# ZooMEISTER/vickers-hardness-Unet

Hardware: AMD Instinct MI355X
Metric: 512x512 images/sec (train fwd+bwd) (higher is better)
Workload: dtype bf16

## Files before the change

include/vk_unet.h:

```cpp
#ifndef VK_UNET_H
#define VK_UNET_H

#include <stddef.h>
#include <stdint.h>

#ifdef __cplusplus
extern "C" {
#endif

#define VK_ABI_VERSION 1
#define VK_STATS_REPLICAS 32

typedef enum { VK_F32 = 0, VK_BF16 = 1, VK_F16 = 2 } vk_dtype;

enum { VK_OK = 0, VK_ERR_ARG = -1, VK_ERR_STATE = -2, VK_ERR_UNSUPPORTED = -3 };

int vk_version(void);
const char* vk_last_error_string(void);
int vk_has_gfx950_code(void);
int vk_probe_mfma_rate(int iters, int waves_per_simd, float* sink, double* flops_out, void* stream);
int vk_set_reserved_cus(int n);
int vk_debug_hold_cus(int workgroups, int threads, int lds_bytes, int microseconds, const void* traffic, size_t traffic_bytes,
                      float* sink, void* stream);

// ... 331 lines not shown
int vk_unet_encoder(const vk_unet* h);
void vk_unet_destroy(vk_unet* h);
int vk_unet_set_side_stream(vk_unet* h, int enable);
int vk_unet_num_tensors(const vk_unet* h);
int vk_unet_tensor_info(const vk_unet* h, int index, vk_tensor_info* out);
int64_t vk_unet_param_numel(const vk_unet* h);
int64_t vk_unet_buffer_numel(const vk_unet* h);
int64_t vk_unet_workspace_bytes(const vk_unet* h);
int vk_unet_num_buckets(const vk_unet* h);
int vk_unet_bucket_range(const vk_unet* h, int bucket, int64_t* elem_begin, int64_t* elem_end);

int vk_unet_bind(vk_unet* h, float* params, float* grads, float* bn_buffers, int64_t* nbt, void* workspace,
                 size_t workspace_bytes);
int vk_unet_refresh_weights(vk_unet* h, void* stream);

int vk_unet_forward(vk_unet* h, const float* x, float* logits, int training, void* stream);
int vk_unet_loss(vk_unet* h, const float* logits, const float* target, float* loss_out, float grad_scale,
                 float w_bce, float w_dice, void* stream);
#define VK_LOSS_BINARY 0
#define VK_LOSS_MULTILABEL 1
#define VK_LOSS_MULTICLASS 2
int vk_unet_loss_ex(vk_unet* h, int mode, const void* logits, const void* target, float* loss_out, float grad_scale, float w_ce,
                    float w_dice, void* stream);
int vk_unet_loss_cfg(vk_unet* h, const vk_seg_loss_cfg* cfg, const void* logits, const void* target, float* loss_out,
                     float grad_scale, void* stream);
int vk_unet_loss_lovasz(vk_unet* h, const vk_seg_loss_cfg* seg_cfg, const vk_lovasz_cfg* lovasz_cfg, float w_lovasz, const void* logits,
                        const void* target, void* workspace, size_t workspace_bytes, float* loss_out, float grad_scale, void* stream);
int vk_unet_backward(vk_unet* h, const float* dlogits, int stage_begin, int stage_end, void* stream);
int vk_unet_set_trainable(vk_unet* h, const uint8_t* flags, int n);
int vk_unet_set_bn_frozen(vk_unet* h, const uint8_t* flags, int n);
// ... 19 lines not shown
```

vickers-hardness-unet_amd/_lib.py:

```python
from __future__ import annotations

import ctypes as C
import os
import subprocess
from pathlib import Path

PKG_DIR = Path(__file__).resolve().parent
LIB_PATH = Path(os.environ["VK_LIB"]) if os.environ.get("VK_LIB") else PKG_DIR / "libvkunet.so"
CSRC = PKG_DIR / "csrc"

VK_F32, VK_BF16, VK_F16 = 0, 1, 2
VK_LOSS_BINARY, VK_LOSS_MULTILABEL, VK_LOSS_MULTICLASS = 0, 1, 2
VK_ENC_RESNET18, VK_ENC_RESNET34, VK_ENC_RESNET50 = 18, 34, 50
VK_ADAMW_MAX_GROUPS = 8
VK_NORM_L2, VK_NORM_INF = 0, 1
VK_TILE_MAX_ORIGINS, VK_TILE_MAX_SIDE = 64, 4096
VK_BLEND_PROB, VK_BLEND_LOGIT = 0, 1


class VkError(RuntimeError):
    pass


class vk_src(C.Structure):
    _fields_ = [("ptr", C.c_void_p), ("C", C.c_int), ("up", C.c_int), ("scale", C.c_void_p),
                ("shift", C.c_void_p), ("relu", C.c_int)]


class vk_conv_desc(C.Structure):
    _fields_ = [("dtype", C.c_int), ("N", C.c_int), ("H", C.c_int), ("W", C.c_int), ("Ho", C.c_int),
# ... 44 lines not shown
    _fields_ = [("struct_size", C.c_uint32), ("mode", C.c_int32), ("terms", C.c_uint32), ("has_ignore", C.c_int32),
                ("ignore_index", C.c_int32), ("w_pix", C.c_float), ("w_focal", C.c_float), ("w_dice", C.c_float),
                ("w_jaccard", C.c_float), ("w_tversky", C.c_float), ("pix_smooth", C.c_float), ("pix_denom_valid", C.c_int32),
                ("has_pos_weight", C.c_int32), ("pos_weight", C.c_float * 16), ("focal_has_alpha", C.c_int32),
                ("focal_alpha", C.c_float), ("focal_gamma", C.c_float),
                ("dice_smooth", C.c_float), ("dice_eps", C.c_float), ("dice_log", C.c_int32), ("dice_classes", C.c_uint32),
                ("jaccard_smooth", C.c_float), ("jaccard_eps", C.c_float), ("jaccard_log", C.c_int32), ("jaccard_classes", C.c_uint32),
                ("tversky_smooth", C.c_float), ("tversky_eps", C.c_float), ("tversky_log", C.c_int32), ("tversky_classes", C.c_uint32),
                ("tversky_alpha", C.c_float), ("tversky_beta", C.c_float), ("tversky_gamma", C.c_float),
                ("w_mcc", C.c_float), ("mcc_eps", C.c_float)]


class vk_lovasz_cfg(C.Structure):
    _fields_ = [("struct_size", C.c_uint32), ("mode", C.c_int32), ("per_image", C.c_int32), ("has_ignore", C.c_int32),
                ("ignore_index", C.c_int32)]


class vk_adamw_group(C.Structure):
    _fields_ = [("lr", C.c_float), ("beta1", C.c_float), ("beta2", C.c_float), ("eps", C.c_float), ("weight_decay", C.c_float)]


class vk_unet_config(C.Structure):
    _fields_ = [("N", C.c_int), ("size", C.c_int), ("dtype", C.c_int), ("training", C.c_int), ("width", C.c_int)]


class vk_tensor_info(C.Structure):
    _fields_ = [("name", C.c_char * 96), ("kind", C.c_int), ("dims", C.c_int * 4), ("ndim", C.c_int),
                ("offset", C.c_int64), ("numel", C.c_int64)]


# ... 89 lines not shown
    "vk_unet_create_ex": (ci, [P(vk_unet_config), ci, P(vp)]),
    "vk_unet_num_classes": (ci, [vp]),
    "vk_unet_create_enc": (ci, [P(vk_unet_config), ci, ci, P(vp)]),
    "vk_unet_encoder": (ci, [vp]),
    "vk_unet_destroy": (None, [vp]),
    "vk_unet_set_side_stream": (ci, [vp, ci]),
    "vk_unet_num_tensors": (ci, [vp]),
    "vk_unet_tensor_info": (ci, [vp, ci, P(vk_tensor_info)]),
    "vk_unet_param_numel": (i64, [vp]),
    "vk_unet_buffer_numel": (i64, [vp]),
    "vk_unet_workspace_bytes": (i64, [vp]),
    "vk_unet_num_buckets": (ci, [vp]),
    "vk_unet_bucket_range": (ci, [vp, ci, P(i64), P(i64)]),
    "vk_unet_bind": (ci, [vp, vp, vp, vp, vp, vp, sz]),
    "vk_unet_refresh_weights": (ci, [vp, vp]),
    "vk_unet_forward": (ci, [vp, vp, vp, ci, vp]),
    "vk_unet_loss": (ci, [vp, vp, vp, vp, cf, cf, cf, vp]),
    "vk_unet_loss_ex": (ci, [vp, ci, vp, vp, vp, cf, cf, cf, vp]),
    "vk_unet_loss_cfg": (ci, [vp, P(vk_seg_loss_cfg), vp, vp, vp, cf, vp]),
    "vk_unet_loss_lovasz": (ci, [vp, P(vk_seg_loss_cfg), P(vk_lovasz_cfg), cf, vp, vp, vp, sz, vp, cf, vp]),
    "vk_unet_backward": (ci, [vp, vp, ci, ci, vp]),
    "vk_unet_set_trainable": (ci, [vp, P(C.c_uint8), ci]),
    "vk_unet_set_bn_frozen": (ci, [vp, P(C.c_uint8), ci]),
    "vk_unet_set_input_grad": (ci, [vp, vp]),
    "vk_unet_zero_grad": (ci, [vp, vp]),
    "vk_unet_debug_tensor": (ci, [vp, C.c_char_p, P(vp), P(ci * 4)]),
    "vk_comm_unique_id": (ci, [vp]),
    "vk_comm_init": (ci, [ci, ci, vp, P(vp)]),
    "vk_comm_world": (ci, [vp]),
    "vk_allreduce_bucket": (ci, [vp, vp, sz, vp]),
# ... 76 lines not shown
```

vickers-hardness-unet_amd/csrc/elementwise.hip:

```cpp
#include <math.h>

#include "vk_common.h"

namespace vk {

static inline int grid_for(size_t work_items, int block = 256, int max_blocks = 256 * 16) {
  size_t b = (work_items + block - 1) / block;
  if (b > (size_t)max_blocks) b = max_blocks;
  if (b < 1) b = 1;
  return (int)b;
}

constexpr int kWideC = 2048;
static inline int channel_grid(int blocks, int cv) {
  int g = cv, r = 256;
  while (r) { const int t = g % r; g = r; r = t; }
  const int m = cv / g;
  return (blocks + m - 1) / m * m;
}

template <typename T>
__global__ void k_input_transform(int N, int H, int W, const float* __restrict__ x, T* __restrict__ x4) {
  const size_t HW = (size_t)H * W;
  const float* xn = x + (size_t)blockIdx.y * 3 * HW;
// ... 1584 lines not shown
  dim3 grid(grid_for(n)), block(256);
  if (!lowp_copy || lowp_dtype == VK_F32) {
    hipLaunchKernelGGL(k_adamw_dev<float>, grid, block, 0, st, n, param, grad, exp_avg, exp_avg_sq, lr, beta1, beta2, eps, weight_decay,
                       (const float*)scratch4, (float*)nullptr);
  } else if (lowp_dtype == VK_BF16) {
    hipLaunchKernelGGL(k_adamw_dev<bf16_t>, grid, block, 0, st, n, param, grad, exp_avg, exp_avg_sq, lr, beta1, beta2, eps, weight_decay,
                       (const float*)scratch4, (bf16_t*)lowp_copy);
  } else {
    hipLaunchKernelGGL(k_adamw_dev<f16_t>, grid, block, 0, st, n, param, grad, exp_avg, exp_avg_sq, lr, beta1, beta2, eps, weight_decay,
                       (const float*)scratch4, (f16_t*)lowp_copy);
  }
  VK_CHECK_HIP(hipGetLastError());
  return VK_OK;
}

extern "C" int vk_adamw_segment_blocks(int n_segments, const int64_t* seg, int32_t* blocks, int capacity) {
  VK_CHECK_ARG(n_segments >= 1 && seg && (capacity >= 0), "vk_adamw_segment_blocks: bad argument");
  int64_t rows = 0;
  for (int s = 0; s < n_segments; ++s) {
    const int64_t b = seg[3 * s], e = seg[3 * s + 1];
    VK_CHECK_ARG(0 <= b && b < e && seg[3 * s + 2] >= 0, "vk_adamw_segment_blocks: bad segment %d [%lld, %lld)", s, (long long)b, (long long)e);
    const int64_t chunks = (e - b + VK_ADAMW_SEGMENT_CHUNK - 1) / VK_ADAMW_SEGMENT_CHUNK;
    for (int64_t c = 0; c < chunks; ++c, ++rows) {
      VK_CHECK_ARG(rows < (1 << 30), "vk_adamw_segment_blocks: too many blocks");
      if (blocks && rows < capacity) {
        blocks[2 * rows] = s;
        blocks[2 * rows + 1] = (int32_t)c;
      }
    }
  }
// ... 36 lines not shown
```

vickers-hardness-unet_amd/csrc/engine.hip:

```cpp
#include <stdarg.h>
#include <stdio.h>
#include <stdlib.h>
#include <string.h>

#include <algorithm>
#include <atomic>
#include <map>
#include <mutex>
#include <string>
#include <vector>

#include "vk_common.h"

namespace vkh {
static thread_local char g_err[512] = "";
void set_error(const char* fmt, ...) {
  va_list ap;
  va_start(ap, fmt);
  vsnprintf(g_err, sizeof(g_err), fmt, ap);
  va_end(ap);
}

struct ProfRec {
  std::string tag;
// ... 221 lines not shown
template <typename T>
__global__ void k_cast_ranges(const CastRange* __restrict__ tab, const float* __restrict__ src, T* __restrict__ dst) {
  const CastRange r = tab[blockIdx.y];
  for (int64_t i = blockIdx.x * (int64_t)blockDim.x + threadIdx.x; i < r.count; i += (int64_t)gridDim.x * blockDim.x)
    st1(dst + r.begin + i, src[r.begin + i]);
}

template <typename T>
__global__ void k_pack_stem(const float* __restrict__ w, T* __restrict__ wp) {
  const int i = blockIdx.x * blockDim.x + threadIdx.x;
  if (i >= 64 * 7 * 32) return;
  const int j = i % 32, r = (i / 32) % 7, k = i / (32 * 7);
  const int s = j >> 2, c = j & 3;
  const float v = (s < 7 && c < 3) ? w[((k * 7 + r) * 7 + s) * 3 + c] : 0.f;
  st1(wp + i, v);
}

struct BnEvalEntry {
  int64_t g_off, b_off, rm_off, rv_off, out_off;
  int C, pad_;
};
__global__ void k_bn_eval_all(const BnEvalEntry* __restrict__ tab, const float* __restrict__ params, const float* __restrict__ bufs,
                              float* __restrict__ arena, float eps) {
  const BnEvalEntry e = tab[blockIdx.x];
  for (int c = threadIdx.x; c < e.C; c += blockDim.x) {
    const float invstd = (float)(1.0 / sqrt((double)bufs[e.rv_off + c] + (double)eps));
    const float sc = params[e.g_off + c] * invstd;
    arena[e.out_off + c] = sc;
    arena[e.out_off + e.C + c] = params[e.b_off + c] - bufs[e.rm_off + c] * sc;
  }
// ... 160 lines not shown
  struct WPlan {
    bool built = false;
    int target = 0, n = 0;
    unsigned version = 0;
    vk::WgradBatchPlan plan;
  };
  std::vector<WItem> pending;
  WPlan wplans[kMaxStages][2];
  size_t off_tab_wbatch = 0;
  std::vector<PackEntry> pack_tab;
  std::vector<CastRange> cast_tab;
  size_t off_tab_cast = 0;
  size_t off_gscratch = 0;
  size_t off_sloss = 0, sloss_bytes = 0;
  size_t off_mloss = 0, mloss_bytes = 0;
  std::vector<BnEvalEntry> bn_tab;
  std::map<std::string, std::pair<void*, std::vector<int>>> debug;

  int N() const { return cfg.N; }
};

namespace {

size_t align_up(size_t v, size_t a) { return (v + a - 1) / a * a; }

bool need_from(const vk_unet* h, int rank) { return h->last_rank >= rank; }
bool trains(const vk_unet* h, int t) { return h->trainable[(size_t)t] != 0; }
bool frozen(const vk_unet* h, const BnL& b) { return (h->bn_frozen_fwd >> b.idx) & 1ull; }
bool bn_sums_needed(const vk_unet* h, const BnL& b) { return !frozen(h, b) || trains(h, b.g_t) || trains(h, b.b_t); }
float* grad_or_sink(vk_unet* h, int t, int64_t off, int sink_off) {
  return trains(h, t) ? h->grads + off : (float*)(h->ws + h->off_gscratch) + sink_off;
}
float* dgamma_of(vk_unet* h, const BnL& b) { return grad_or_sink(h, b.g_t, b.g_off, 0); }
float* dbeta_of(vk_unet* h, const BnL& b) { return grad_or_sink(h, b.b_t, b.b_off, h->sink_c); }

// ... 250 lines not shown
  h->off_wstem = take(64 * 7 * 32 * eb);
  h->off_wslab = tr ? take(kEngineSlabBytes) : 0;
  h->off_tab_wbatch = tr ? take((size_t)kMaxStages * 2 * VK_WGRAD_BATCH_TABLE_BYTES) : 0;
  h->splitk_bytes = (!tr && (size_t)N * S * SW <= 4u * 512 * 512) ? VK_SPLITK_WORKSPACE_BYTES : 0;
  h->off_splitk = h->splitk_bytes ? take(h->splitk_bytes) : 0;
  h->off_tab_pack = take(h->convs.size() * sizeof(PackEntry));
  h->off_tab_cast = take(h->convs.size() * sizeof(CastRange));
  h->off_tab_bn = take(h->bns.size() * sizeof(BnEvalEntry));
  h->off_gscratch = tr ? take(grad_scratch_floats(h) * sizeof(float)) : 0;
  if (h->classes > 1) {
    h->mloss_bytes = vk_multi_loss_workspace_bytes(N, h->classes, S * SW);
    h->off_mloss = take(h->mloss_bytes);
  }
  h->sloss_bytes = vk_seg_loss_workspace_bytes(N, h->classes, S * SW);
  h->off_sloss = take(h->sloss_bytes);
  h->ws_bytes = off;
}

void assign_pointers(vk_unet* h) {
  char* ws = h->ws;
  h->debug.clear();
  const int N = h->cfg.N;
  for (size_t i = 0; i < h->convs.size(); ++i) {
    ConvL& c = h->convs[i];
    if ((int)i == h->head_conv) continue;
    c.z = ws + h->off_z[i];
    c.g = h->cfg.training ? ws + h->off_g[i] : nullptr;
    h->debug["z:" + c.name] = {c.z, {N, c.Hout, c.Wout, c.K}};
    if (c.g) h->debug["g:" + c.name] = {c.g, {N, c.Hout, c.Wout, c.K}};
  }
// ... 174 lines not shown
  VK_CHECK_ARG(h && out && index >= 0 && index < (int)h->infos.size(), "vk_unet_tensor_info: bad index %d", index);
  *out = h->infos[index];
  return VK_OK;
}
extern "C" int64_t vk_unet_param_numel(const vk_unet* h) { return h ? h->n_params : 0; }
extern "C" int64_t vk_unet_buffer_numel(const vk_unet* h) { return h ? h->n_bufs : 0; }
extern "C" int64_t vk_unet_workspace_bytes(const vk_unet* h) { return h ? (int64_t)h->ws_bytes : 0; }
extern "C" int vk_unet_num_buckets(const vk_unet* h) { return h ? (int)h->buckets.size() : 0; }
extern "C" int vk_unet_bucket_range(const vk_unet* h, int bucket, int64_t* b, int64_t* e) {
  VK_CHECK_ARG(h && b && e && bucket >= 0 && bucket < (int)h->buckets.size(), "vk_unet_bucket_range: bad bucket %d", bucket);
  *b = h->buckets[bucket].first;
  *e = h->buckets[bucket].second;
  return VK_OK;
}

extern "C" int vk_unet_bind(vk_unet* h, float* params, float* grads, float* bn_buffers, int64_t* nbt, void* workspace,
                            size_t workspace_bytes) {
  VK_CHECK_ARG(h && params && bn_buffers && nbt && workspace, "vk_unet_bind: null argument");
  VK_CHECK_ARG(!h->cfg.training || grads, "vk_unet_bind: a training plan needs a gradient buffer");
  VK_CHECK_ARG(workspace_bytes >= h->ws_bytes, "vk_unet_bind: workspace too small (%zu < %zu)", workspace_bytes, h->ws_bytes);
  VK_CHECK_ARG(((uintptr_t)workspace & 255) == 0 && ((uintptr_t)params & 15) == 0, "vk_unet_bind: buffers must be 256-byte (workspace) / 16-byte (params) aligned");
  h->params = params; h->grads = grads; h->bufs = bn_buffers; h->nbt = nbt; h->ws = (char*)workspace;
  for (auto& st_ : h->wplans) { st_[0].built = false; st_[1].built = false; }
  h->pending.clear();
  assign_pointers(h);
  h->halo_tab.clear();
  {
    auto plain = [&](int C) { vk_src s = null_src(); s.ptr = h->ws; s.C = C; return s; };
    auto fwd_uses = [&](ConvL& c, int C0, int C1, int up) {
      vk_src s0 = plain(C0), s1 = C1 ? plain(C1) : null_src();
      s0.up = up;
      vk_conv_desc d = conv_desc(h, c, s0, s1);
      return vk_conv_uses_halo_pack(&d) != 0;
    };
    for (size_t i = 0; i < h->convs.size(); ++i) {
      ConvL& c = h->convs[i];
      c.halo_fwd = c.halo_dg = false;
      if ((int)i == h->stem_conv || (int)i == h->head_conv) continue;
      c.halo_fwd = fwd_uses(c, c.Cin, 0, 0);
    }
    for (DecL& d : h->decs) {
      ConvL& c = h->convs[d.conv1];
      c.halo_fwd = fwd_uses(c, d.Cup, d.Cskip, 1);
    }
    for (size_t i = 0; i < h->convs.size(); ++i) {
      ConvL& c = h->convs[i];
      if (c.wd_off >= 0 && h->cfg.training) {
        vk_conv_desc d;
        d.dtype = h->cfg.dtype;
        d.N = h->cfg.N; d.H = c.Hout; d.W = c.Wout; d.Ho = c.Hin; d.Wo = c.Win;
        d.K = c.Cin; d.R = c.R; d.S = c.R; d.stride = c.stride; d.pad = c.pad; d.transposed = 1;
        d.src0 = plain(c.K);
        d.src1 = null_src();
        c.halo_dg = vk_conv_uses_halo_pack(&d) != 0;
      }
      HaloPackEntry e;
      e.src = c.w_off; e.pad_ = 0;
      if (c.halo_fwd) {
        e.dst = (int64_t)(h->off_wh + (size_t)c.w_off * h->eb); e.rows = c.K; e.red = c.Cin; e.transposed = 0;
        h->halo_tab.push_back(e);
      }
      if (c.halo_dg) {
        e.dst = (int64_t)(h->off_wd + (size_t)c.wd_off * h->eb); e.rows = c.Cin; e.red = c.K; e.transposed = 1;
        h->halo_tab.push_back(e);
      }
    }
  }
  h->pack_tab.clear();
  for (size_t i = 0; i < h->convs.size(); ++i) {
    const ConvL& c = h->convs[i];
    if (c.wd_off < 0 || c.halo_dg) continue;
    PackEntry e;
    e.src = c.w_off; e.dst = c.wd_off; e.K = c.K; e.RS = c.R * c.R; e.C = c.Cin; e.pad_ = 0;
    h->pack_tab.push_back(e);
  }
  h->cast_tab.clear();
  for (size_t i = 0; i < h->convs.size(); ++i) {
    const ConvL& c = h->convs[i];
    if ((int)i == h->stem_conv || (int)i == h->head_conv || c.halo_fwd) continue;
    h->cast_tab.push_back(CastRange{c.w_off, (int64_t)c.K * c.Cin * c.R * c.R});
  }
  h->bn_tab.clear();
  for (const BnL& b : h->bns) {
    BnEvalEntry e;
    e.g_off = b.g_off; e.b_off = b.b_off; e.rm_off = b.rm_off; e.rv_off = b.rv_off; e.out_off = b.arena_off; e.C = b.C; e.pad_ = 0;
    h->bn_tab.push_back(e);
  }
  if (!h->pack_tab.empty())
    VK_CHECK_HIP(hipMemcpy(h->ws + h->off_tab_pack, h->pack_tab.data(), h->pack_tab.size() * sizeof(PackEntry), hipMemcpyHostToDevice));
  if (!h->halo_tab.empty())
    VK_CHECK_HIP(hipMemcpy(h->ws + h->off_tab_halo, h->halo_tab.data(), h->halo_tab.size() * sizeof(HaloPackEntry), hipMemcpyHostToDevice));
  if (!h->cast_tab.empty())
    VK_CHECK_HIP(hipMemcpy(h->ws + h->off_tab_cast, h->cast_tab.data(), h->cast_tab.size() * sizeof(CastRange), hipMemcpyHostToDevice));
  VK_CHECK_HIP(hipMemcpy(h->ws + h->off_tab_bn, h->bn_tab.data(), h->bn_tab.size() * sizeof(BnEvalEntry), hipMemcpyHostToDevice));
  if (h->cfg.training && !h->side && getenv("VK_SIDE_STREAM")) RET_IF(vk_unet_set_side_stream(h, 1));
  h->bound = true;
  return VK_OK;
}

template <typename T>
static int refresh_t(vk_unet* h, hipStream_t st) {
  vkh::ProfScope ps_("weights_repack", st, 0.0, (double)h->n_params * (4.0 + 2.0 * sizeof(T)));
  if (sizeof(T) != 4 && !h->cast_tab.empty())
    hipLaunchKernelGGL(k_cast_ranges<T>, dim3(16, (unsigned)h->cast_tab.size()), dim3(256), 0, st, (const CastRange*)(h->ws + h->off_tab_cast),
                       h->params, (T*)(h->ws + h->off_wf));
  if (h->cfg.training && !h->pack_tab.empty())
    hipLaunchKernelGGL(k_pack_dgrad<T>, dim3(64, (unsigned)h->pack_tab.size()), dim3(256), 0, st,
                       (const PackEntry*)(h->ws + h->off_tab_pack), h->params, (T*)(h->ws + h->off_wd));
  if (!h->halo_tab.empty())
// ... 2 lines not shown
  hipLaunchKernelGGL(k_pack_stem<T>, dim3((64 * 7 * 32 + 255) / 256), dim3(256), 0, st,
                     h->params + h->convs[h->stem_conv].w_off, (T*)(h->ws + h->off_wstem));
  VK_CHECK_HIP(hipGetLastError());
  return VK_OK;
}

extern "C" int vk_unet_refresh_weights(vk_unet* h, void* stream) {
  VK_CHECK_ARG(h && h->bound, "vk_unet_refresh_weights: plan not bound");
  hipStream_t st = (hipStream_t)stream;
  switch (h->cfg.dtype) {
    case VK_F32: return refresh_t<float>(h, st);
    case VK_BF16: return refresh_t<bf16_t>(h, st);
    case VK_F16: return refresh_t<f16_t>(h, st);
  }
  return VK_ERR_ARG;
}

extern "C" int vk_unet_set_side_stream(vk_unet* h, int enable) {
  VK_CHECK_ARG(h, "vk_unet_set_side_stream: null plan");
  if (enable && !h->side && h->cfg.training) {
    VK_CHECK_HIP(hipStreamCreateWithFlags(&h->side, hipStreamNonBlocking));
    VK_CHECK_HIP(hipEventCreateWithFlags(&h->ev_fork, hipEventDisableTiming));
    VK_CHECK_HIP(hipEventCreateWithFlags(&h->ev_join, hipEventDisableTiming));
  } else if (!enable && h->side) {
    VK_CHECK_HIP(hipStreamSynchronize(h->side));
    (void)hipEventDestroy(h->ev_fork);
    (void)hipEventDestroy(h->ev_join);
    (void)hipStreamDestroy(h->side);
    h->side = nullptr;
    h->ev_fork = h->ev_join = nullptr;
// ... 647 lines not shown
```

vickers-hardness-unet_amd/csrc/vk_common.h:

```cpp
#pragma once
#include <hip/hip_runtime.h>
#include <stdint.h>

#include "../../include/vk_unet.h"

namespace vk {

struct bf16_t { uint16_t v; };
struct f16_t  { uint16_t v; };

typedef __attribute__((ext_vector_type(8))) __bf16   bf16x8_t;
typedef __attribute__((ext_vector_type(8))) _Float16 f16x8_t;
typedef __attribute__((ext_vector_type(4))) float    f32x4_t;
typedef __attribute__((ext_vector_type(4))) uint32_t u32x4_t;
typedef __attribute__((ext_vector_type(2))) uint32_t u32x2_t;
typedef __attribute__((ext_vector_type(4))) short    s16x4_t;
typedef __attribute__((ext_vector_type(2))) float    f32x2_t;
typedef __attribute__((ext_vector_type(2))) __bf16   bf16x2_t;
typedef __attribute__((ext_vector_type(2))) _Float16 f16x2_t;
typedef __attribute__((ext_vector_type(2))) short    s16x2_t;

template <typename T> struct ElemTraits;
template <> struct ElemTraits<float> {
  static constexpr int kBytes = 4;
// ... 225 lines not shown
                                            float bc2_sqrt, float inv_scale) {
#pragma clang fp contract(off)
  const float gr = g[i];
  const float gi = gr * inv_scale;
  const float keep = __builtin_fmaf(-lr, wd, 1.f);
  float mi = m[i];
  mi = __builtin_fmaf(__builtin_fmaf(gr, inv_scale, -mi), 1.f - beta1, mi);
  const float vi = __builtin_fmaf(gi, (1.f - beta2) * gi, v[i] * beta2);
  const float denom = sqrtf(vi) / bc2_sqrt + eps;
  const float pi = __builtin_fmaf(p[i], keep, -(step_size * (mi / denom)));
  p[i] = pi;
  m[i] = mi;
  v[i] = vi;
  return pi;
}

}

namespace vkh {
inline vk::FastDiv make_fastdiv(uint32_t d) {
  vk::FastDiv f;
  f.div = d;
  if (d <= 1) { f.mul = 0; f.shr = 0; f.div = 1; return f; }
  uint32_t lg = 0;
  while ((1u << lg) < d) ++lg;
  uint32_t p = 31 + lg;
  f.mul = (uint32_t)(((1ull << p) + d - 1) / d);
  f.shr = p - 32;
  return f;
}
void set_error(const char* fmt, ...);
int reserved_cus();

struct ProfScope {
  int idx;
  hipStream_t st;
  hipEvent_t ev_end;
  ProfScope(const char* tag, hipStream_t stream, double flops, double bytes);
  ~ProfScope();
};
}

#define VK_CHECK_ARG(cond, ...)                \
  do {                                         \
    if (!(cond)) {                             \
      vkh::set_error(__VA_ARGS__);             \
// ... 26 lines not shown
```

vickers-hardness-unet_amd/optim.py:

```python
from __future__ import annotations

import ctypes as C
import math
from typing import Dict, List, Optional, Tuple

import torch

from . import _lib
from ._lib import VkError, check, lib


class FusedAdamW(torch.optim.Optimizer):
    _step_supports_amp_scaling = True

    def __init__(self, params, lr: float = 1e-3, betas=(0.9, 0.999), eps: float = 1e-8, weight_decay: float = 1e-2,
                 amsgrad: bool = False):
        if amsgrad:
            raise NotImplementedError("amsgrad is not used by the reference")
        params = list(params)
        if not params:
            raise VkError("FusedAdamW takes model.parameters() of one vickers-hardness-unet_amd.Unet, a subset of them, or a list of "
                          "param-group dicts over them")
        defaults = dict(lr=lr, betas=betas, eps=eps, weight_decay=weight_decay)
        self._model = None
# ... 118 lines not shown
        if gs is not None and not isinstance(gs, torch.Tensor):
            raise VkError("grad_scale must be a device tensor (a float here would have to come from a host sync)")
        if fi is not None:
            fi = fi.reshape(-1)[:1].to(device=p.device, dtype=torch.float32)
        if gs is not None:
            gs = gs.reshape(-1)[:1].to(device=p.device, dtype=torch.float32)
        if len(self.param_groups) > 1 or clip is not None:
            self._step_groups(m, active, gs, fi, clip)
            m.mark_weights_dirty()
            return None
        grp = self.param_groups[0]
        if len(active) < len(m._param_list) or self._steps_dev is not None:
            self._step_segments(m, active, grp, gs, fi)
            m.mark_weights_dirty()
            return None
        check(lib().vk_adamw_step_amp(p.numel(), p.data_ptr(), g.data_ptr(), self._m.data_ptr(), self._v.data_ptr(),
                                      float(grp["lr"]), float(grp["betas"][0]), float(grp["betas"][1]), float(grp["eps"]),
                                      float(grp["weight_decay"]), self._step_dev.data_ptr(), float(self.grad_inv_scale),
                                      _lib.ptr(gs), _lib.ptr(fi), self._scratch.data_ptr(), 0, 0, _lib.current_stream()),
              "vk_adamw_step_amp")
        m.mark_weights_dirty()
        return None

    def _tables(self, m, active: Tuple[int, ...]):
        dev = m.flat_params.device
        L = lib()
        if self._seg_key != (active, dev):
            seg = torch.tensor([[m._param_ranges[t][0], m._param_ranges[t][0] + m._param_ranges[t][1], t] for t in active],
                               dtype=torch.int64)
            seg_p = C.cast(seg.data_ptr(), C.POINTER(C.c_int64))
# ... 129 lines not shown
```

vickers-hardness-unet_amd/unet.py:

```python
from __future__ import annotations

import os
import ctypes as C
import math
from typing import Dict, List, Optional, Tuple

import torch
import torch.nn as nn

from . import _lib
from ._lib import VkError, check, lib


class _Holder(nn.Module):

    def forward(self, *a, **k):
        raise RuntimeError("structural container only; call the Unet")


class _Plan:

    def __init__(self, model: "Unet", N: int, S, dtype: torch.dtype, training: bool):
        L = lib()
        H, W = (S, S) if isinstance(S, int) else S
# ... 133 lines not shown
                check(L.vk_unet_tensor_info(h, i, C.byref(ti)))
                self._table.append((ti.name.decode(), ti.kind, [ti.dims[j] for j in range(ti.ndim)], ti.offset, ti.numel))
            n_params = L.vk_unet_param_numel(h)
            n_bufs = L.vk_unet_buffer_numel(h)
        finally:
            L.vk_unet_destroy(h)
        n_bn = sum(1 for t in self._table if t[1] == 3)
        self._flat: Dict[str, Optional[torch.Tensor]] = {
            "params": torch.zeros(n_params, dtype=torch.float32),
            "grads": None,
            "bufs": torch.zeros(n_bufs, dtype=torch.float32),
            "nbt": torch.zeros(n_bn, dtype=torch.int64),
        }
        self._leaves: Dict[str, Tuple[nn.Module, str]] = {}
        self._plans: Dict[tuple, _Plan] = {}
        self._dirty = 0
        self._reducer = None
        self._time_groups = None
        self._group_events = []
        self._anchor = torch.zeros((), requires_grad=True)
        self._build_tree()
        self._rebuild_views()
        self._default_init()

    def _create_handle(self, cfg, h):
        if self.encoder_name == "resnet34":
            check(lib().vk_unet_create_ex(C.byref(cfg), self.classes, C.byref(h)), "vk_unet_create_ex")
        else:
            code = {"resnet18": _lib.VK_ENC_RESNET18, "resnet50": _lib.VK_ENC_RESNET50}[self.encoder_name]
            check(lib().vk_unet_create_enc(C.byref(cfg), self.classes, code, C.byref(h)), "vk_unet_create_enc")
# ... 38 lines not shown
        self._param_ranges = [(t[3], t[4]) for t in self._table if t[1] in (0, 1)]
        self._bn_modules = [self._leaves[t[0]][0] for t in self._table if t[1] == 3]

    def _apply(self, fn, recurse=True):
        for k in ("params", "grads", "bufs", "nbt"):
            t = self._flat[k]
            if t is not None:
                nt = fn(t)
                want = torch.int64 if k == "nbt" else torch.float32
                if nt.dtype != want:
                    raise VkError("the fp32 master copy cannot be converted to %s; choose the compute type with "
                                  "torch.autocast or compute_dtype=" % nt.dtype)
                self._flat[k] = nt
        self._rebuild_views()
        self._plans.clear()
        self._dirty += 1
        return self

    def _default_init(self):
        sd = {name: self._view(kind, dims, off, numel) for name, kind, dims, off, numel in self._table}

        def ctor_draw(shape, bias=False):
            w = torch.empty(shape)
            nn.init.kaiming_uniform_(w, a=math.sqrt(5))
            if bias:
                fan_in = w[0].numel()
                bound = 1 / math.sqrt(fan_in)
                nn.init.uniform_(torch.empty(shape[0]), -bound, bound)

        with torch.no_grad():
# ... 96 lines not shown
            raise RuntimeError(f"Wrong input shape height={h}, width={w}. Expected image height and width divisible by 32.")
        if not x.is_cuda:
            raise VkError("input is on %s: this package runs on an MI355X only and has no CPU fallback" % x.device)
        if self._flat["params"].device != x.device:
            raise VkError("model is on %s but the input is on %s" % (self._flat["params"].device, x.device))

    def _run_forward(self, plan: _Plan, x: torch.Tensor, training: bool) -> torch.Tensor:
        L = lib()
        st = _lib.current_stream()
        ver = self._weights_version()
        if plan.weights_version != ver:
            check(L.vk_unet_refresh_weights(plan.h, st), "vk_unet_refresh_weights")
            plan.weights_version = ver
        x = x.detach().contiguous().float()
        if training:
            plan.set_bn_frozen(self._bn_frozen_flags())
        logits = torch.empty(plan.N, self.classes, plan.H, plan.W, dtype=torch.float32, device=x.device)
        check(L.vk_unet_forward(plan.h, x.data_ptr(), logits.data_ptr(), 1 if training else 0, st), "vk_unet_forward")
        plan._last_x = x
        return logits

    def _run_backward(self, plan: _Plan, dlogits: Optional[torch.Tensor], mask: Tuple[bool, ...], want_dx: bool = False):
        L = lib()
        st = _lib.current_stream()
        plan.set_trainable(self, mask)
        plan.set_input_grad(want_dx, self._flat["params"].device)
        if all(mask):
            fresh = next(iter(self.parameters())).grad is None
        else:
            fresh = all(p.grad is None for p, t in zip(self._param_list, mask) if t)
# ... 175 lines not shown
```

Baseline: 3123.

## Fuse AdamW update with bf16 forward and dgrad weight repacking

Result: no change. 3144, median of 6 (+0.7%).

```diff
diff --git a/include/vk_unet.h b/include/vk_unet.h
--- a/include/vk_unet.h
+++ b/include/vk_unet.h
@@ -369,6 +369,19 @@
                  size_t workspace_bytes);
 int vk_unet_refresh_weights(vk_unet* h, void* stream);
 
+int vk_unet_adamw_step(vk_unet* h, float* exp_avg, float* exp_avg_sq, float lr, float beta1, float beta2, float eps,
+                       float weight_decay, int* step_count, float inv_scale, const float* grad_scale, const float* found_inf,
+                       float* scratch4, void* stream);
+enum { VK_APK_PLAIN = 0, VK_APK_TILE = 1, VK_APK_STEM = 2 };
+typedef struct vk_adamw_pack_item {
+  int64_t src, fwd_dst, dg_dst;
+  int32_t kind, count, first;
+  int32_t K, RS, C, k0, c0, kb, cb;
+  int32_t fwd, dg;
+} vk_adamw_pack_item;
+int vk_unet_adamw_pack_table(vk_unet* h, vk_adamw_pack_item* items_host, int capacity);
+int vk_unet_weight_pack_regions(const vk_unet* h, int64_t out[8]);
+
 int vk_unet_forward(vk_unet* h, const float* x, float* logits, int training, void* stream);
 int vk_unet_loss(vk_unet* h, const float* logits, const float* target, float* loss_out, float grad_scale,
                  float w_bce, float w_dice, void* stream);
diff --git a/vickers-hardness-unet_amd/_lib.py b/vickers-hardness-unet_amd/_lib.py
--- a/vickers-hardness-unet_amd/_lib.py
+++ b/vickers-hardness-unet_amd/_lib.py
@@ -14,6 +14,8 @@
 VK_ENC_RESNET18, VK_ENC_RESNET34, VK_ENC_RESNET50 = 18, 34, 50
 VK_ADAMW_MAX_GROUPS = 8
 VK_NORM_L2, VK_NORM_INF = 0, 1
+VK_OK, VK_ERR_UNSUPPORTED = 0, -3
+VK_APK_PLAIN, VK_APK_TILE, VK_APK_STEM = 0, 1, 2
 VK_TILE_MAX_ORIGINS, VK_TILE_MAX_SIDE = 64, 4096
 VK_BLEND_PROB, VK_BLEND_LOGIT = 0, 1
 
@@ -88,6 +90,12 @@
 class vk_lovasz_cfg(C.Structure):
     _fields_ = [("struct_size", C.c_uint32), ("mode", C.c_int32), ("per_image", C.c_int32), ("has_ignore", C.c_int32),
                 ("ignore_index", C.c_int32)]
+
+
+class vk_adamw_pack_item(C.Structure):
+    _fields_ = [("src", C.c_int64), ("fwd_dst", C.c_int64), ("dg_dst", C.c_int64), ("kind", C.c_int32), ("count", C.c_int32),
+                ("first", C.c_int32), ("K", C.c_int32), ("RS", C.c_int32), ("C", C.c_int32), ("k0", C.c_int32), ("c0", C.c_int32),
+                ("kb", C.c_int32), ("cb", C.c_int32), ("fwd", C.c_int32), ("dg", C.c_int32)]
 
 
 class vk_adamw_group(C.Structure):
@@ -207,6 +215,9 @@
     "vk_unet_bucket_range": (ci, [vp, ci, P(i64), P(i64)]),
     "vk_unet_bind": (ci, [vp, vp, vp, vp, vp, vp, sz]),
     "vk_unet_refresh_weights": (ci, [vp, vp]),
+    "vk_unet_adamw_step": (ci, [vp, vp, vp, cf, cf, cf, cf, cf, vp, cf, vp, vp, vp, vp]),
+    "vk_unet_adamw_pack_table": (ci, [vp, P(vk_adamw_pack_item), ci]),
+    "vk_unet_weight_pack_regions": (ci, [vp, P(i64)]),
     "vk_unet_forward": (ci, [vp, vp, vp, ci, vp]),
     "vk_unet_loss": (ci, [vp, vp, vp, vp, cf, cf, cf, vp]),
     "vk_unet_loss_ex": (ci, [vp, ci, vp, vp, vp, cf, cf, cf, vp]),
diff --git a/vickers-hardness-unet_amd/csrc/elementwise.hip b/vickers-hardness-unet_amd/csrc/elementwise.hip
--- a/vickers-hardness-unet_amd/csrc/elementwise.hip
+++ b/vickers-hardness-unet_amd/csrc/elementwise.hip
@@ -1622,6 +1622,11 @@
   return VK_OK;
 }
 
+void vkh::adamw_prepare(hipStream_t st, int* step_count, const float* grad_scale, const float* found_inf, float lr, float beta1,
+                        float beta2, float inv_scale, float* scratch4) {
+  hipLaunchKernelGGL(k_adamw_prepare, dim3(1), dim3(64), 0, st, step_count, grad_scale, found_inf, lr, beta1, beta2, inv_scale, scratch4);
+}
+
 extern "C" int vk_adamw_segment_blocks(int n_segments, const int64_t* seg, int32_t* blocks, int capacity) {
   VK_CHECK_ARG(n_segments >= 1 && seg && (capacity >= 0), "vk_adamw_segment_blocks: bad argument");
   int64_t rows = 0;
diff --git a/vickers-hardness-unet_amd/csrc/engine.hip b/vickers-hardness-unet_amd/csrc/engine.hip
--- a/vickers-hardness-unet_amd/csrc/engine.hip
+++ b/vickers-hardness-unet_amd/csrc/engine.hip
@@ -259,6 +259,109 @@
   const int s = j >> 2, c = j & 3;
   const float v = (s < 7 && c < 3) ? w[((k * 7 + r) * 7 + s) * 3 + c] : 0.f;
   st1(wp + i, v);
+}
+
+constexpr int kApkTileElems = 32 * 9 * 32;
+template <typename T>
+__global__ __launch_bounds__(256) void k_adamw_pack(const vk_adamw_pack_item* __restrict__ tab, float* __restrict__ p,
+                                                    const float* __restrict__ g, float* __restrict__ m, float* __restrict__ v,
+                                                    char* __restrict__ ws, float lr, float beta1, float beta2, float eps, float wd,
+                                                    const float* __restrict__ st) {
+  static_assert(sizeof(T) == 2, "the packs of an fp32 plan are the master weights themselves");
+  if (st[0] != 0.f) return;
+  const float step_size = st[1], bc2_sqrt = st[2], inv_scale = st[3];
+  __shared__ __attribute__((aligned(16))) uint16_t tile[kApkTileElems];
+  const vk_adamw_pack_item e = tab[blockIdx.x];
+  const int tid = threadIdx.x;
+  if (e.kind != VK_APK_TILE) {
+    T* stem = reinterpret_cast<T*>(ws + e.fwd_dst);
+    for (int i = tid; i < e.count; i += 256) {
+      const int64_t idx = e.src + i;
+      float pi = p[idx], mi = m[idx], vi = v[idx];
+      adamw_vals(pi, g[idx], mi, vi, lr, beta1, beta2, eps, wd, step_size, bc2_sqrt, inv_scale);
+      p[idx] = pi;
+      m[idx] = mi;
+      v[idx] = vi;
+      if (e.kind == VK_APK_STEM) {
+        const int j = e.first + i;
+        const int c = j % 3, s = (j / 3) % 7, kr = j / 21;
+        st1(stem + kr * 32 + s * 4 + c, pi);
+      }
+    }
+    return;
+  }
+  const int RS = e.RS, C = e.C, K = e.K, CB = e.cb, KB = e.kb;
+  const int cq_shift = CB == 32 ? 3 : 2;
+  const int rows = KB * RS;
+  const int64_t base = e.src + (int64_t)e.k0 * RS * C + e.c0;
+  for (int q = tid; q < (rows << cq_shift); q += 256) {
+    const int row = q >> cq_shift, col = (q & ((1 << cq_shift) - 1)) * 4;
+    const int64_t idx = base + (int64_t)row * C + col;
+    f32x4_t p4 = *reinterpret_cast<const f32x4_t*>(p + idx);
+    const f32x4_t g4 = *reinterpret_cast<const f32x4_t*>(g + idx);
+    f32x4_t m4 = *reinterpret_cast<const f32x4_t*>(m + idx);
+    f32x4_t v4 = *reinterpret_cast<const f32x4_t*>(v + idx);
+    float pf[4], mf[4], vf[4];
+#pragma unroll
+    for (int i = 0; i < 4; ++i) {
+      pf[i] = p4[i]; mf[i] = m4[i]; vf[i] = v4[i];
+      adamw_vals(pf[i], g4[i], mf[i], vf[i], lr, beta1, beta2, eps, wd, step_size, bc2_sqrt, inv_scale);
+      p4[i] = pf[i]; m4[i] = mf[i]; v4[i] = vf[i];
+    }
+    *reinterpret_cast<f32x4_t*>(p + idx) = p4;
+    *reinterpret_cast<f32x4_t*>(m + idx) = m4;
+    *reinterpret_cast<f32x4_t*>(v + idx) = v4;
+    T* t4 = reinterpret_cast<T*>(tile + row * CB + col);
+#pragma unroll
+    for (int i = 0; i < 4; ++i) st1(t4 + i, pf[i]);
+  }
+  __syncthreads();
+  if (e.fwd == 1) {
+    const int cv_shift = cq_shift - 1;
+    for (int x = tid; x < (rows << cv_shift); x += 256) {
+      const int row = x >> cv_shift, c8 = (x & ((1 << cv_shift) - 1)) * 8;
+      const int64_t off = ((int64_t)e.k0 * RS + row) * C + e.c0 + c8;
+      *reinterpret_cast<u32x4_t*>(ws + e.fwd_dst + off * 2) = *reinterpret_cast<const u32x4_t*>(tile + row * CB + c8);
+    }
+  } else if (e.fwd == 2) {
+    u32x4_t* dst = reinterpret_cast<u32x4_t*>(ws + e.fwd_dst);
+    const int cc = e.c0 >> 5;
+    for (int x = tid; x < rows * 4; x += 256) {
+      const int pos = x & 3, kl = (x >> 2) % KB, tap = (x >> 2) / KB;
+      const int k = e.k0 + kl;
+      const int j = pos ^ (((k >> 2) & 1) << 1);
+      dst[(((int64_t)cc * 9 + tap) * K + k) * 4 + pos] = *reinterpret_cast<const u32x4_t*>(tile + (kl * 9 + tap) * 32 + j * 8);
+    }
+  }
+  if (e.dg == 1) {
+    const int kvn = KB >> 3;
+    for (int x = tid; x < CB * RS * kvn; x += 256) {
+      const int kv = x % kvn, cl = (x / kvn) % CB, t = x / (kvn * CB);
+      u32x4_t o;
+#pragma unroll
+      for (int i = 0; i < 4; ++i) {
+        const uint32_t lo = tile[((kv * 8 + 2 * i) * RS + t) * CB + cl], hi = tile[((kv * 8 + 2 * i + 1) * RS + t) * CB + cl];
+        o[i] = lo | (hi << 16);
+      }
+      const int64_t off = ((int64_t)(e.c0 + cl) * RS + t) * K + e.k0 + kv * 8;
+      *reinterpret_cast<u32x4_t*>(ws + e.dg_dst + off * 2) = o;
+    }
+  } else if (e.dg == 2) {
+    u32x4_t* dst = reinterpret_cast<u32x4_t*>(ws + e.dg_dst);
+    const int kc = e.k0 >> 5;
+    for (int x = tid; x < CB * 9 * 4; x += 256) {
+      const int pos = x & 3, cl = (x >> 2) % CB, tap = (x >> 2) / CB;
+      const int c = e.c0 + cl;
+      const int j = pos ^ (((c >> 2) & 1) << 1);
+      u32x4_t o;
+#pragma unroll
+      for (int i = 0; i < 4; ++i) {
+        const uint32_t lo = tile[((j * 8 + 2 * i) * 9 + tap) * CB + cl], hi = tile[((j * 8 + 2 * i + 1) * 9 + tap) * CB + cl];
+        o[i] = lo | (hi << 16);
+      }
+      dst[(((int64_t)kc * 9 + tap) * C + c) * 4 + pos] = o;
+    }
+  }
 }
 
 struct BnEvalEntry {
@@ -449,11 +552,16 @@
   size_t off_gscratch = 0;
   size_t off_sloss = 0, sloss_bytes = 0;
   size_t off_mloss = 0, mloss_bytes = 0;
+  std::vector<vk_adamw_pack_item> apk_tab;
+  size_t off_tab_apk = 0, apk_capacity = 0;
+  double apk_bytes = 0;
   std::vector<BnEvalEntry> bn_tab;
   std::map<std::string, std::pair<void*, std::vector<int>>> debug;
 
   int N() const { return cfg.N; }
 };
+
+static bool build_apk_items(const vk_unet* h, std::vector<vk_adamw_pack_item>& out, double* pack_bytes);
 
 namespace {
 
@@ -734,6 +842,11 @@
   }
   h->sloss_bytes = vk_seg_loss_workspace_bytes(N, h->classes, S * SW);
   h->off_sloss = take(h->sloss_bytes);
+  {
+    std::vector<vk_adamw_pack_item> tab;
+    h->apk_capacity = build_apk_items(h, tab, nullptr) ? tab.size() : 0;
+    h->off_tab_apk = h->apk_capacity ? take(h->apk_capacity * sizeof(vk_adamw_pack_item)) : 0;
+  }
   h->ws_bytes = off;
 }
 
@@ -938,6 +1051,120 @@
   return VK_OK;
 }
 
+static void decide_halo_routes(vk_unet* h, const void* any) {
+  auto plain = [&](int C) { vk_src s = null_src(); s.ptr = const_cast<void*>(any); s.C = C; return s; };
+  auto fwd_uses = [&](ConvL& c, int C0, int C1, int up) {
+    vk_src s0 = plain(C0), s1 = C1 ? plain(C1) : null_src();
+    s0.up = up;
+    vk_conv_desc d = conv_desc(h, c, s0, s1);
+    return vk_conv_uses_halo_pack(&d) != 0;
+  };
+  for (size_t i = 0; i < h->convs.size(); ++i) {
+    ConvL& c = h->convs[i];
+    c.halo_fwd = c.halo_dg = false;
+    if ((int)i == h->stem_conv || (int)i == h->head_conv) continue;
+    c.halo_fwd = fwd_uses(c, c.Cin, 0, 0);
+  }
+  for (DecL& d : h->decs) {
+    ConvL& c = h->convs[d.conv1];
+    c.halo_fwd = fwd_uses(c, d.Cup, d.Cskip, 1);
+  }
+  for (size_t i = 0; i < h->convs.size(); ++i) {
+    ConvL& c = h->convs[i];
+    if (c.wd_off >= 0 && h->cfg.training) {
+      vk_conv_desc d;
+      d.dtype = h->cfg.dtype;
+      d.N = h->cfg.N; d.H = c.Hout; d.W = c.Wout; d.Ho = c.Hin; d.Wo = c.Win;
+      d.K = c.Cin; d.R = c.R; d.S = c.R; d.stride = c.stride; d.pad = c.pad; d.transposed = 1;
+      d.src0 = plain(c.K);
+      d.src1 = null_src();
+      c.halo_dg = vk_conv_uses_halo_pack(&d) != 0;
+    }
+  }
+}
+
+static bool build_apk_items(const vk_unet* h, std::vector<vk_adamw_pack_item>& out, double* pack_bytes) {
+  out.clear();
+  double pb = 0;
+  if (!h->cfg.training || h->eb != 2) return false;
+  auto item = [](int kind, int64_t src, int count) {
+    vk_adamw_pack_item e;
+    memset(&e, 0, sizeof(e));
+    e.kind = kind; e.src = src; e.count = count;
+    return e;
+  };
+  auto plain = [&](int64_t b, int64_t e_) {
+    for (; b < e_; b += VK_ADAMW_SEGMENT_CHUNK) out.push_back(item(VK_APK_PLAIN, b, (int)std::min<int64_t>(VK_ADAMW_SEGMENT_CHUNK, e_ - b)));
+  };
+  int64_t cursor = 0;
+  for (size_t i = 0; i < h->convs.size(); ++i) {
+    const ConvL& c = h->convs[i];
+    if ((int)i == h->head_conv) continue;
+    const int RS = c.R * c.R;
+    const int64_t numel = (int64_t)c.K * RS * c.Cin;
+    if (c.w_off < cursor) return false;
+    plain(cursor, c.w_off);
+    cursor = c.w_off + numel;
+    if ((int)i == h->stem_conv) {
+      if (c.K != 64 || c.R != 7 || c.Cin != 3) return false;
+      for (int64_t b = 0; b < numel; b += VK_ADAMW_SEGMENT_CHUNK) {
+        vk_adamw_pack_item e = item(VK_APK_STEM, c.w_off + b, (int)std::min<int64_t>(VK_ADAMW_SEGMENT_CHUNK, numel - b));
+        e.first = (int)b;
+        e.fwd_dst = (int64_t)h->off_wstem;
+        out.push_back(e);
+      }
+      pb += (double)numel * 2;
+      continue;
+    }
+    const int kb = std::min(32, c.K), cb = std::min(32, c.Cin);
+    if (c.K % kb || c.Cin % cb || (cb != 16 && cb != 32) || kb % 8 || kb * RS * cb > kApkTileElems || c.w_off % 4) return false;
+    vk_adamw_pack_item e = item(VK_APK_TILE, c.w_off, kb * RS * cb);
+    e.K = c.K; e.RS = RS; e.C = c.Cin; e.kb = kb; e.cb = cb;
+    if (c.halo_fwd) {
+      if (cb != 32 || RS != 9) return false;
+      e.fwd = 2; e.fwd_dst = (int64_t)(h->off_wh + (size_t)c.w_off * 2);
+    } else {
+      if (c.w_off % 8) return false;
+      e.fwd = 1; e.fwd_dst = (int64_t)(h->off_wf + (size_t)c.w_off * 2);
+    }
+    pb += (double)numel * 2;
+    if (c.wd_off >= 0) {
+      if (c.halo_dg && (kb != 32 || RS != 9)) return false;
+      if (c.wd_off % 8) return false;
+      e.dg = c.halo_dg ? 2 : 1;
+      e.dg_dst = (int64_t)(h->off_wd + (size_t)c.wd_off * 2);
+      pb += (double)numel * 2;
+    }
+    for (e.k0 = 0; e.k0 < c.K; e.k0 += kb)
+      for (e.c0 = 0; e.c0 < c.Cin; e.c0 += cb) out.push_back(e);
+  }
+  plain(cursor, h->n_params);
+  std::stable_sort(out.begin(), out.end(), [](const vk_adamw_pack_item& a, const vk_adamw_pack_item& b) { return a.count > b.count; });
+  if (pack_bytes) *pack_bytes = pb;
+  return true;
+}
+
+extern "C" int vk_unet_adamw_pack_table(vk_unet* h, vk_adamw_pack_item* items_host, int capacity) {
+  VK_CHECK_ARG(h && capacity >= 0, "vk_unet_adamw_pack_table: bad argument");
+  if (!h->cfg.training || h->eb != 2) return VK_ERR_UNSUPPORTED;
+  if (!h->bound) decide_halo_routes(h, h);
+  std::vector<vk_adamw_pack_item> tab;
+  if (!build_apk_items(h, tab, nullptr)) return VK_ERR_UNSUPPORTED;
+  if (items_host)
+    for (size_t i = 0; i < tab.size() && i < (size_t)capacity; ++i) items_host[i] = tab[i];
+  return (int)tab.size();
+}
+
+extern "C" int vk_unet_weight_pack_regions(const vk_unet* h, int64_t out[8]) {
+  VK_CHECK_ARG(h && out, "vk_unet_weight_pack_regions: null argument");
+  const int64_t eb = h->eb;
+  out[0] = (int64_t)h->off_wf;    out[1] = eb == 4 ? 0 : h->n_params * eb;
+  out[2] = (int64_t)h->off_wd;    out[3] = h->cfg.training ? h->n_dgrad * eb : 0;
+  out[4] = (int64_t)h->off_wh;    out[5] = h->n_params * eb;
+  out[6] = (int64_t)h->off_wstem; out[7] = 64 * 7 * 32 * eb;
+  return VK_OK;
+}
+
 extern "C" int vk_unet_bind(vk_unet* h, float* params, float* grads, float* bn_buffers, int64_t* nbt, void* workspace,
                             size_t workspace_bytes) {
   VK_CHECK_ARG(h && params && bn_buffers && nbt && workspace, "vk_unet_bind: null argument");
@@ -948,46 +1175,19 @@
   for (auto& st_ : h->wplans) { st_[0].built = false; st_[1].built = false; }
   h->pending.clear();
   assign_pointers(h);
+  decide_halo_routes(h, h->ws);
   h->halo_tab.clear();
-  {
-    auto plain = [&](int C) { vk_src s = null_src(); s.ptr = h->ws; s.C = C; return s; };
-    auto fwd_uses = [&](ConvL& c, int C0, int C1, int up) {
-      vk_src s0 = plain(C0), s1 = C1 ? plain(C1) : null_src();
-      s0.up = up;
-      vk_conv_desc d = conv_desc(h, c, s0, s1);
-      return vk_conv_uses_halo_pack(&d) != 0;
-    };
-    for (size_t i = 0; i < h->convs.size(); ++i) {
-      ConvL& c = h->convs[i];
-      c.halo_fwd = c.halo_dg = false;
-      if ((int)i == h->stem_conv || (int)i == h->head_conv) continue;
-      c.halo_fwd = fwd_uses(c, c.Cin, 0, 0);
-    }
-    for (DecL& d : h->decs) {
-      ConvL& c = h->convs[d.conv1];
-      c.halo_fwd = fwd_uses(c, d.Cup, d.Cskip, 1);
-    }
-    for (size_t i = 0; i < h->convs.size(); ++i) {
-      ConvL& c = h->convs[i];
-      if (c.wd_off >= 0 && h->cfg.training) {
-        vk_conv_desc d;
-        d.dtype = h->cfg.dtype;
-        d.N = h->cfg.N; d.H = c.Hout; d.W = c.Wout; d.Ho = c.Hin; d.Wo = c.Win;
-        d.K = c.Cin; d.R = c.R; d.S = c.R; d.stride = c.stride; d.pad = c.pad; d.transposed = 1;
-        d.src0 = plain(c.K);
-        d.src1 = null_src();
-        c.halo_dg = vk_conv_uses_halo_pack(&d) != 0;
-      }
-      HaloPackEntry e;
-      e.src = c.w_off; e.pad_ = 0;
-      if (c.halo_fwd) {
-        e.dst = (int64_t)(h->off_wh + (size_t)c.w_off * h->eb); e.rows = c.K; e.red = c.Cin; e.transposed = 0;
-        h->halo_tab.push_back(e);
-      }
-      if (c.halo_dg) {
-        e.dst = (int64_t)(h->off_wd + (size_t)c.wd_off * h->eb); e.rows = c.Cin; e.red = c.K; e.transposed = 1;
-        h->halo_tab.push_back(e);
-      }
+  for (size_t i = 0; i < h->convs.size(); ++i) {
+    const ConvL& c = h->convs[i];
+    HaloPackEntry e;
+    e.src = c.w_off; e.pad_ = 0;
+    if (c.halo_fwd) {
+      e.dst = (int64_t)(h->off_wh + (size_t)c.w_off * h->eb); e.rows = c.K; e.red = c.Cin; e.transposed = 0;
+      h->halo_tab.push_back(e);
+    }
+    if (c.halo_dg) {
+      e.dst = (int64_t)(h->off_wd + (size_t)c.wd_off * h->eb); e.rows = c.Cin; e.red = c.K; e.transposed = 1;
+      h->halo_tab.push_back(e);
     }
   }
   h->pack_tab.clear();
@@ -1017,6 +1217,10 @@
   if (!h->cast_tab.empty())
     VK_CHECK_HIP(hipMemcpy(h->ws + h->off_tab_cast, h->cast_tab.data(), h->cast_tab.size() * sizeof(CastRange), hipMemcpyHostToDevice));
   VK_CHECK_HIP(hipMemcpy(h->ws + h->off_tab_bn, h->bn_tab.data(), h->bn_tab.size() * sizeof(BnEvalEntry), hipMemcpyHostToDevice));
+  if (!build_apk_items(h, h->apk_tab, &h->apk_bytes) || h->apk_tab.size() > h->apk_capacity) h->apk_tab.clear();
+  h->apk_bytes += 28.0 * (double)h->n_params;
+  if (!h->apk_tab.empty())
+    VK_CHECK_HIP(hipMemcpy(h->ws + h->off_tab_apk, h->apk_tab.data(), h->apk_tab.size() * sizeof(vk_adamw_pack_item), hipMemcpyHostToDevice));
   if (h->cfg.training && !h->side && getenv("VK_SIDE_STREAM")) RET_IF(vk_unet_set_side_stream(h, 1));
   h->bound = true;
   return VK_OK;
@@ -1049,6 +1253,31 @@
     case VK_F16: return refresh_t<f16_t>(h, st);
   }
   return VK_ERR_ARG;
+}
+
+namespace {
+int join_side(vk_unet* h, hipStream_t st);
+}
+
+extern "C" int vk_unet_adamw_step(vk_unet* h, float* exp_avg, float* exp_avg_sq, float lr, float beta1, float beta2, float eps,
+                                  float weight_decay, int* step_count, float inv_scale, const float* grad_scale, const float* found_inf,
+                                  float* scratch4, void* stream) {
+  VK_CHECK_ARG(h && exp_avg && exp_avg_sq && step_count && scratch4, "vk_unet_adamw_step: bad argument");
+  if (!h->bound || !h->cfg.training || h->eb != 2 || !h->grads || h->apk_tab.empty() || getenv("VK_NO_ADAMW_PACK")) return VK_ERR_UNSUPPORTED;
+  hipStream_t st = (hipStream_t)stream;
+  RET_IF(join_side(h, st));
+  vkh::adamw_prepare(st, step_count, grad_scale, found_inf, lr, beta1, beta2, inv_scale, scratch4);
+  vkh::ProfScope ps_("adamw_pack", st, 0.0, h->apk_bytes);
+  const vk_adamw_pack_item* tab = (const vk_adamw_pack_item*)(h->ws + h->off_tab_apk);
+  const dim3 grid((unsigned)h->apk_tab.size()), block(256);
+  if (h->cfg.dtype == VK_BF16)
+    hipLaunchKernelGGL(k_adamw_pack<bf16_t>, grid, block, 0, st, tab, h->params, (const float*)h->grads, exp_avg, exp_avg_sq, h->ws, lr, beta1,
+                       beta2, eps, weight_decay, (const float*)scratch4);
+  else
+    hipLaunchKernelGGL(k_adamw_pack<f16_t>, grid, block, 0, st, tab, h->params, (const float*)h->grads, exp_avg, exp_avg_sq, h->ws, lr, beta1,
+                       beta2, eps, weight_decay, (const float*)scratch4);
+  VK_CHECK_HIP(hipGetLastError());
+  return VK_OK;
 }
 
 extern "C" int vk_unet_set_side_stream(vk_unet* h, int enable) {
diff --git a/vickers-hardness-unet_amd/csrc/vk_common.h b/vickers-hardness-unet_amd/csrc/vk_common.h
--- a/vickers-hardness-unet_amd/csrc/vk_common.h
+++ b/vickers-hardness-unet_amd/csrc/vk_common.h
@@ -263,6 +263,18 @@
   v[i] = vi;
   return pi;
 }
+__device__ __forceinline__ void adamw_vals(float& p, float gr, float& m, float& v, float lr, float beta1, float beta2, float eps, float wd,
+                                           float step_size, float bc2_sqrt, float inv_scale) {
+#pragma clang fp contract(off)
+  const float gi = gr * inv_scale;
+  const float keep = __builtin_fmaf(-lr, wd, 1.f);
+  const float mi = __builtin_fmaf(__builtin_fmaf(gr, inv_scale, -m), 1.f - beta1, m);
+  const float vi = __builtin_fmaf(gi, (1.f - beta2) * gi, v * beta2);
+  const float denom = sqrtf(vi) / bc2_sqrt + eps;
+  p = __builtin_fmaf(p, keep, -(step_size * (mi / denom)));
+  m = mi;
+  v = vi;
+}
 
 }
 
@@ -279,6 +291,8 @@
   return f;
 }
 void set_error(const char* fmt, ...);
+void adamw_prepare(hipStream_t st, int* step_count, const float* grad_scale, const float* found_inf, float lr, float beta1, float beta2,
+                   float inv_scale, float* scratch4);
 int reserved_cus();
 
 struct ProfScope {
diff --git a/vickers-hardness-unet_amd/optim.py b/vickers-hardness-unet_amd/optim.py
--- a/vickers-hardness-unet_amd/optim.py
+++ b/vickers-hardness-unet_amd/optim.py
@@ -156,6 +156,18 @@
             self._step_segments(m, active, grp, gs, fi)
             m.mark_weights_dirty()
             return None
+        plan = getattr(m, "_train_plan", None)
+        if plan is not None and plan.weights_version == m._weights_version() and plan.ws.device == p.device:
+            rc = lib().vk_unet_adamw_step(plan.h, self._m.data_ptr(), self._v.data_ptr(), float(grp["lr"]), float(grp["betas"][0]),
+                                          float(grp["betas"][1]), float(grp["eps"]), float(grp["weight_decay"]),
+                                          self._step_dev.data_ptr(), float(self.grad_inv_scale), _lib.ptr(gs), _lib.ptr(fi),
+                                          self._scratch.data_ptr(), _lib.current_stream())
+            if rc == _lib.VK_OK:
+                m.mark_weights_dirty()
+                plan.weights_version = m._weights_version()
+                return None
+            if rc != _lib.VK_ERR_UNSUPPORTED:
+                check(rc, "vk_unet_adamw_step")
         check(lib().vk_adamw_step_amp(p.numel(), p.data_ptr(), g.data_ptr(), self._m.data_ptr(), self._v.data_ptr(),
                                       float(grp["lr"]), float(grp["betas"][0]), float(grp["betas"][1]), float(grp["eps"]),
                                       float(grp["weight_decay"]), self._step_dev.data_ptr(), float(self.grad_inv_scale),
diff --git a/vickers-hardness-unet_amd/unet.py b/vickers-hardness-unet_amd/unet.py
--- a/vickers-hardness-unet_amd/unet.py
+++ b/vickers-hardness-unet_amd/unet.py
@@ -171,6 +171,7 @@
         }
         self._leaves: Dict[str, Tuple[nn.Module, str]] = {}
         self._plans: Dict[tuple, _Plan] = {}
+        self._train_plan: Optional[_Plan] = None
         self._dirty = 0
         self._reducer = None
         self._time_groups = None
@@ -239,6 +240,7 @@
                 self._flat[k] = nt
         self._rebuild_views()
         self._plans.clear()
+        self._train_plan = None
         self._dirty += 1
         return self
 
@@ -365,6 +367,8 @@
             plan.weights_version = ver
         x = x.detach().contiguous().float()
         if training:
+            if plan.training:
+                self._train_plan = plan
             plan.set_bn_frozen(self._bn_frozen_flags())
         logits = torch.empty(plan.N, self.classes, plan.H, plan.W, dtype=torch.float32, device=x.device)
         check(L.vk_unet_forward(plan.h, x.data_ptr(), logits.data_ptr(), 1 if training else 0, st), "vk_unet_forward")
```
